# dpkn31/Yade-OpenFOAM-coupling

Hardware: AMD Instinct MI355X
Metric: coupled_steps_per_sec (pimpleFoamYade 4-way, 10M particles / 4M cells per GPU) (higher is better)
Workload: dtype f64

## Files before the change

yade-openfoam-coupling_amd/csrc/common.hpp:

```cpp
#pragma once
#include <hip/hip_runtime.h>

#include <algorithm>
#include <cmath>
#include <cstdarg>
#include <cstdint>
#include <cstdio>
#include <cstring>
#include <string>
#include <vector>

#include "../../include/foamyade_hip.h"

namespace fy {

struct Options {
    std::string tree_cache_dir;
    int rebin_interval;
    int strip_blocks;
    bool halo_overlap;
    int ipc_slot_mb;
    long long ipc_timeout_ms;
    bool wire_trace;
    bool explicit_tree;
    bool no_locate_lists;
    int locate_stack;
    bool locate_wide;
    bool no_deep_vcycle;
    long long mg_replicate_below;
    int amg_passes;
    bool localcomm_stream;
    bool no_fused_corrector;
    bool faces_from_arrays;
    bool no_pairs;
    bool no_tail_cache;
    int ipc_slot_kb;
};
Options options();

std::string& last_error();
int fail(int code, const char* fmt, ...);
bool pairs_disabled();
bool tail_cache_disabled();
bool locate_wide_forced();

#define FY_HIP(expr)                                                                                      \
    do {                                                                                                  \
        hipError_t _e = (expr);                                                                           \
        if (_e != hipSuccess)                                                                             \
            return ::fy::fail(FY_ERR_HIP, "%s failed: %s (%s:%d)", #expr, hipGetErrorString(_e), __FILE__, __LINE__); \
    } while (0)

#define FY_TRY(expr)                 \
    do {                             \
        int _rc = (expr);            \
        if (_rc != FY_OK) return _rc; \
// ... 203 lines not shown
```

yade-openfoam-coupling_amd/csrc/coupling.cpp:

```cpp
#include "coupling.hpp"
#include "ldu.hpp"

#include <algorithm>
#include <cmath>
#include <chrono>
#include <cstdlib>
#include <functional>
#include <thread>

#include <sys/stat.h>
#include <unistd.h>

#include <atomic>

namespace fy {

static std::atomic<int> g_kernel_flags{-1};
static bool kernel_flag(int bit) {
    if (g_kernel_flags.load(std::memory_order_relaxed) < 0) (void)options();
    return (g_kernel_flags.load(std::memory_order_relaxed) >> bit) & 1;
}
bool pairs_disabled() { return kernel_flag(0); }
bool tail_cache_disabled() { return kernel_flag(1); }
bool locate_wide_forced() { return kernel_flag(2); }

Options options() {
    auto on = [](const char* nm) { const char* e = getenv(nm); return e != nullptr && *e != 0 && strcmp(e, "0") != 0; };
    auto num = [](const char* nm, long long unset) { const char* e = getenv(nm); return e ? atoll(e) : unset; };
    Options q{};
    if (const char* d = getenv("FOAMYADE_TREE_CACHE_DIR")) q.tree_cache_dir = d;
    q.rebin_interval = std::max(1, (int)num("FOAMYADE_REBIN_INTERVAL", 32));
    q.strip_blocks = (int)num("FOAMYADE_STRIP_BLOCKS", -1);
    q.halo_overlap = getenv("FOAMYADE_HALO_OVERLAP") == nullptr || on("FOAMYADE_HALO_OVERLAP");
    q.ipc_slot_mb = (int)num("FOAMYADE_IPC_SLOT_MB", 0);
    q.ipc_timeout_ms = num("FOAMYADE_IPC_TIMEOUT_MS", 0);
    q.wire_trace = getenv("FOAMYADE_WIRE_TRACE") != nullptr;
    q.explicit_tree = on("FOAMYADE_EXPLICIT_TREE");
    q.no_locate_lists = on("FOAMYADE_NO_LOCATE_LISTS");
    q.locate_stack = (int)num("FOAMYADE_LOCATE_STACK", -1);
    q.locate_wide = num("FOAMYADE_LOCATE_WIDE", 0) != 0;
    q.no_deep_vcycle = on("FOAMYADE_NO_DEEP_VCYCLE");
    q.mg_replicate_below = std::max(0LL, num("FOAMYADE_MG_REPLICATE_BELOW", 0));
    q.amg_passes = (int)std::min(3LL, std::max(1LL, num("FOAMYADE_AMG_PASSES", 3)));
    const char* ls = getenv("FOAMYADE_LOCALCOMM_STREAM");
    q.localcomm_stream = ls != nullptr && ls[0] == '1';
    q.no_fused_corrector = on("FOAMYADE_NO_FUSED_CORRECTOR");
    q.faces_from_arrays = on("FOAMYADE_FACES_FROM_ARRAYS");
    q.no_pairs = on("FOAMYADE_NO_PAIRS");
    q.no_tail_cache = on("FOAMYADE_NO_TAIL_CACHE");
    q.ipc_slot_kb = (int)num("FOAMYADE_IPC_SLOT_KB", 0);
    g_kernel_flags.store((q.no_pairs ? 1 : 0) | (q.no_tail_cache ? 2 : 0) | (q.locate_wide ? 4 : 0), std::memory_order_relaxed);
    return q;
}

std::string& last_error() {
    static thread_local std::string e;
    return e;
}

int fail(int code, const char* fmt, ...) {
    char buf[1024];
    va_list ap;
    va_start(ap, fmt);
    vsnprintf(buf, sizeof(buf), fmt, ap);
    va_end(ap);
    last_error() = buf;
    return code;
}

static const int TAG_SZ_BUFF = 1003, TAG_GRID_BBOX = 1001, TAG_YADE_DATA = 1002, TAG_FORCE = 1005, TAG_SEARCH_RES = 1004,
// ... 1368 lines not shown
```

yade-openfoam-coupling_amd/csrc/fv_kernels.hip:

```cpp
#include "fv_kernels.hpp"

#include "common.hpp"
#include "device_util.hpp"
#include "fv_closures.hpp"

#ifndef FY_FVK_GRADED
#define FY_FVK_GRADED 0
#endif

namespace fy {
#if FY_FVK_GRADED
namespace gr {
#endif
namespace {

constexpr double kSmall = 1e-15;

__device__ __forceinline__ void ijk_of(const FvGeo& g, int t, int& i, int& j, int& k) {
    i = t % g.nx;
    const int q = t / g.nx;
    j = q % g.ny;
    k = q / g.ny;
}
__device__ __forceinline__ int cidx(const FvGeo& g, int i, int j, int k) { return i + g.nx * (j + g.ny * (k + g.gz)); }
// ... 377 lines not shown
    int i, j, k; ijk_of(g, t, i, j, k);
#define FY_CALL(D, fi, fj, fk) { const size_t f = (size_t)fid(g, D, fi, fj, fk); \
        flux_correct_face<D>(g, f, fi, fj, fk, p, phiHbyA.a[D], rAUf.a[D], alphaf.a[D], psn.a[D], phiForces.a[D], pflux.a[D], phi.a[D]); }
    FY_CELL_FACES(g, i, j, k, FY_CALL);
#undef FY_CALL
}

__global__ __launch_bounds__(256) void k_courant(FvGeo g, CFace3 phi, double* __restrict__ partials) {
    double v[2] = {0.0, 0.0};
    FY_RED_LOOP_G(g, t) {
        int i, j, k; ijk_of(g, t, i, j, k);
        double s = 0.0;
#pragma unroll
        for (int d = 0; d < 3; ++d)
#pragma unroll
            for (int sd = 0; sd < 2; ++sd) s += fabs(phi.a[d][cface(g, d, sd, i, j, k)]);
        v[0] = fmax(v[0], s * geo_rV(g, i, j, k));
        v[1] += s;
    }
    const int mx[2] = {1, 0};
    block_reduce_store<2>(v, mx, partials, fy_lb, fy_stride);
}

__global__ __launch_bounds__(256) void k_pre_coupling(FvGeo g, const double* __restrict__ U, const double* __restrict__ p,
                                                      const double* __restrict__ alpha, CFace3 psn, double* __restrict__ vGrad,
                                                      double* __restrict__ gradP, double* __restrict__ divT, double* __restrict__ Gout,
                                                      int write_vgrad, int write_pfields, CFace3 phi, double* __restrict__ ddtU, double* __restrict__ Uold_out,
                                                      double* __restrict__ cellrec, double rec_two_nu, double rec_rhoF, Face3 dcorr) {
    const int t = fv_block(g, blockIdx.x, gridDim.x) * 256 + (int)threadIdx.x;
    if (t >= g.Nc) return;
    int i, j, k; ijk_of(g, t, i, j, k);
    const int c = t + g.c0;
    const bool pf = g.pimple && write_pfields;
    const int ijk[3] = {i, j, k};
    bool bnd[3][2];
#pragma unroll
    for (int d = 0; d < 3; ++d)
#pragma unroll
        for (int s = 0; s < 2; ++s) bnd[d][s] = onb(g, d, s, i, j, k);
    const double uc[3] = {U[3 * (size_t)c], U[3 * (size_t)c + 1], U[3 * (size_t)c + 2]};
    const double pc = pf ? p[c] : 0.0, ac = pf ? alpha[c] : 0.0;
    double un6[3][2][3], pn6[3][2], an6[3][2];
#pragma unroll
    for (int d = 1; d < 3; ++d)
#pragma unroll
        for (int s = 0; s < 2; ++s) {
// ... 8 lines not shown
#pragma unroll
        for (int s = 0; s < 2; ++s) phf[d][s] = want_phi ? phi.a[d][cface(g, d, s, i, j, k)] : 0.0;
    const int lane = threadIdx.x & 63;
    {
        const int xm = (lane == 0 && i > 0) ? c - 1 : c, xp = (lane == 63 && i + 1 < g.nx) ? c + 1 : c;
        double em[3] = {0, 0, 0}, ep[3] = {0, 0, 0}, epm = 0, epp = 0, eam = 0, eap = 0;
        if (lane == 0 || lane == 63) {
            for (int q = 0; q < 3; ++q) { em[q] = U[3 * (size_t)xm + q]; ep[q] = U[3 * (size_t)xp + q]; }
            if (pf) { epm = p[xm]; epp = p[xp]; eam = alpha[xm]; eap = alpha[xp]; }
        }
#pragma unroll
        for (int q = 0; q < 3; ++q) { un6[0][0][q] = wave_prev(uc[q]); un6[0][1][q] = wave_next(uc[q]); }
        pn6[0][0] = wave_prev(pc); pn6[0][1] = wave_next(pc); an6[0][0] = wave_prev(ac); an6[0][1] = wave_next(ac);
        if (lane == 0 && i > 0) { for (int q = 0; q < 3; ++q) un6[0][0][q] = em[q]; pn6[0][0] = epm; an6[0][0] = eam; }
        if (lane == 63 && i + 1 < g.nx) { for (int q = 0; q < 3; ++q) un6[0][1][q] = ep[q]; pn6[0][1] = epp; an6[0][1] = eap; }
    }
    if (Uold_out) { Uold_out[3 * (size_t)c] = uc[0]; Uold_out[3 * (size_t)c + 1] = uc[1]; Uold_out[3 * (size_t)c + 2] = uc[2]; }
    double lap[3] = {0, 0, 0}, T[9], conv[3] = {0, 0, 0}, gp3[3] = {0, 0, 0};
#pragma unroll
    for (int d = 0; d < 3; ++d) {
        double fv[2][3], fp[2] = {0, 0};
#pragma unroll
        for (int s = 0; s < 2; ++s) {
            if (bnd[d][s]) {
                const int patch = 2 * d + s;
                if (g.u_bc[patch] == 0) { fv[s][0] = g.u_val[patch][0]; fv[s][1] = g.u_val[patch][1]; fv[s][2] = g.u_val[patch][2]; }
                else { fv[s][0] = uc[0]; fv[s][1] = uc[1]; fv[s][2] = uc[2]; }
                if (g.u_bc[patch] == 2) fv[s][d] = 0.0;
                if (pf) {
                    fp[s] = pbv(g, p, psn, c, d, s, cface(g, d, s, i, j, k));
                    for (int q = 0; q < 3; ++q) lap[q] += 1.0 * geo_Af(g, d, i, j, k) * (fv[s][q] - uc[q]) * geo_rhalf(g, d, ijk[d]);
                }
            } else {
                const double* un = un6[d][s];
                const int qc = ijk[d];
                for (int q = 0; q < 3; ++q) fv[s][q] = geo_lerp_side(g, d, s, qc, uc[q], un[q]);
                if (pf) {
                    fp[s] = geo_lerp_side(g, d, s, qc, pc, pn6[d][s]);
                    const double af = geo_lerp_side(g, d, s, qc, ac, an6[d][s]);
                    for (int q = 0; q < 3; ++q) lap[q] += af * geo_Af(g, d, i, j, k) * (un[q] - uc[q]) * geo_rdelta(g, d, qc + s);
                }
            }
        }
        if (dcorr.a[0]) {
#pragma unroll
            for (int s = 0; s < 2; ++s)
                if (owns_face(g, d, s, i, j, k)) {
                    const int fi = i + (d == 0 ? s : 0), fj = j + (d == 1 ? s : 0), fk = k + (d == 2 ? s : 0);
                    const int f = cface(g, d, s, i, j, k);
                    const double uf = fv[s][d] * geo_Af(g, d, fi, fj, fk);
                    const double po = phf[d][s];
                    const double phiCorr = po - uf;
                    const bool fixes = bnd[d][s] && g.u_bc[2 * d + s] == 0;
                    const double coef = fixes ? 0.0 : 1.0 - fmin(fabs(phiCorr) / (fabs(po) + kSmall), 1.0);
                    dcorr.a[d][f] = coef * (1.0 / g.dt) * phiCorr;
                }
        }
        const double rhd = geo_rh(g, d, ijk[d]);
        for (int q = 0; q < 3; ++q) T[3 * d + q] = (fv[1][q] - fv[0][q]) * rhd;
        if (pf) gp3[d] = (fp[1] - fp[0]) * rhd;
        if (ddtU) {
#pragma unroll
            for (int s = 0; s < 2; ++s) {
                const double flux = (s ? 1.0 : -1.0) * phf[d][s];
                for (int q = 0; q < 3; ++q) conv[q] += flux * fv[s][q];
            }
        }
    }
    if (ddtU)
        for (int q = 0; q < 3; ++q) ddtU[3 * (size_t)c + q] = conv[q] * geo_rV(g, i, j, k);
    if (write_vgrad)
        for (int q = 0; q < 9; ++q) vGrad[9 * (size_t)c + q] = T[q];
    if (pf)
        for (int q = 0; q < 3; ++q) gradP[3 * (size_t)c + q] = gp3[q];
    if (pf) {
        double dT[3];
        for (int q = 0; q < 3; ++q) { dT[q] = 2 * g.nu * (lap[q] * geo_rV(g, i, j, k)); divT[3 * (size_t)c + q] = dT[q]; }
        if (cellrec) {
            double2* r = reinterpret_cast<double2*>(cellrec + 8 * (size_t)c);
            r[0] = make_double2(uc[0], uc[1]);
            r[1] = make_double2(uc[2], ac);
            r[2] = make_double2(((rec_two_nu * dT[0]) * rec_rhoF) - gp3[0], ((rec_two_nu * dT[1]) * rec_rhoF) - gp3[1]);
            r[3] = make_double2(((rec_two_nu * dT[2]) * rec_rhoF) - gp3[2], geo_V(g, i, j, k));
        }
    }
    if (Gout) {
        const double tr = T[0] + T[4] + T[8];
        const double an = g.nut ? alpha[c] * (g.nu + g.nut[c]) : alpha[c] * g.nu;
        const size_t rs = g_row_stride(g);
        for (int a = 0; a < 3; ++a)
            for (int b = 0; b < 3; ++b) Gout[(size_t)a * rs + 3 * (size_t)c + b] = an * (T[3 * b + a] - (a == b ? (2.0 / 3.0) * tr : 0.0));
    }
}

__global__ __launch_bounds__(256) void k_div_G(FvGeo g, const double* __restrict__ G, double* __restrict__ divG) {
    const int t = fv_block(g, blockIdx.x, gridDim.x) * 256 + (int)threadIdx.x;
    if (t >= g.Nc) return;
    int i, j, k; ijk_of(g, t, i, j, k);
    const int c = t + g.c0;
    const int ijk[3] = {i, j, k};
    const double g0[3] = {G[3 * (size_t)c], G[3 * (size_t)c + 1], G[3 * (size_t)c + 2]};
    double gx[2][3];
    x_neighbours3(G, c, i, g.nx, g0, gx[0], gx[1]);
    bool bnd[3][2];
    double own[3][3], nbv[3][2][3];
#pragma unroll
    for (int q = 0; q < 3; ++q) { own[0][q] = g0[q]; nbv[0][0][q] = gx[0][q]; nbv[0][1][q] = gx[1][q]; }
#pragma unroll
    for (int d = 0; d < 3; ++d)
#pragma unroll
        for (int s = 0; s < 2; ++s) bnd[d][s] = onb(g, d, s, i, j, k);
#pragma unroll
    for (int d = 1; d < 3; ++d) {
        const double* Gd = G + (size_t)d * g_row_stride(g);
#pragma unroll
        for (int q = 0; q < 3; ++q) own[d][q] = Gd[3 * (size_t)c + q];
#pragma unroll
        for (int s = 0; s < 2; ++s) {
            const int nb = bnd[d][s] ? c : c + (s ? stride_of(g, d) : -stride_of(g, d));
#pragma unroll
            for (int q = 0; q < 3; ++q) nbv[d][s][q] = Gd[3 * (size_t)nb + q];
        }
    }
    double acc[3] = {0, 0, 0};
#pragma unroll
    for (int d = 0; d < 3; ++d) {
        double fv[2][3];
#pragma unroll
        for (int s = 0; s < 2; ++s)
            for (int q = 0; q < 3; ++q) fv[s][q] = bnd[d][s] ? own[d][q] : geo_lerp_side(g, d, s, ijk[d], own[d][q], nbv[d][s][q]);
        for (int q = 0; q < 3; ++q) acc[q] += (fv[1][q] - fv[0][q]) * geo_rh(g, d, ijk[d]);
    }
    for (int q = 0; q < 3; ++q) divG[3 * (size_t)c + q] = acc[q];
}

__global__ __launch_bounds__(256) void k_smagorinsky_nut(FvGeo g, const double* __restrict__ vGrad, double ck, double ce, double delta, double* __restrict__ nut) {
    const int t = blockIdx.x * 256 + threadIdx.x;
    if (t >= g.Nc) return;
    const int c = t + g.c0;
    delta = geo_delta(g, delta, c);
    double T[9];
#pragma unroll
    for (int q = 0; q < 9; ++q) T[q] = vGrad[9 * (size_t)c + q];
    nut[c] = smagorinsky_nut(T, ck, ce, delta);
}

__device__ __forceinline__ double wall_epsilon(const FvGeo& g, const TurbEqn& e, double kc, int c, int i, int j, int k) {
#if FY_FVK_GRADED
    double sum = 0.0;
    int W = 0;
#pragma unroll
    for (int d = 0; d < 3; ++d)
#pragma unroll
        for (int s = 0; s < 2; ++s)
            if (e.wall[2 * d + s] && onb(g, d, s, i, j, k)) { sum += wall_epsilon_term(e.cmu75, kc, e.kappa, geo_ywall(g, d, c)); ++W; }
// ... 949 lines not shown
}

int launch_pre_coupling(hipStream_t s, FvGeo g, const double* U, const double* p, const double* alpha, CFace3 psn, double* vGrad,
                        double* gradP, double* divT, double* Gout, int write_vgrad, int write_pfields, CFace3 phi, double* ddtU, double* Uold_out,
                        double* cellrec, double rec_nu, double rec_rhoF, Face3 dcorr) {
    hipLaunchKernelGGL(k_pre_coupling, dim3(fv_grid(g)), dim3(256), 0, s, g, U, p, alpha, psn, vGrad, gradP, divT, Gout, write_vgrad, write_pfields,
                       phi, ddtU, Uold_out, cellrec, 2.0 * rec_nu, rec_rhoF, dcorr);
    FY_LAUNCH_CHECK();
    return FY_OK;
}

int launch_interp_alpha(hipStream_t s, FvGeo g, const double* alpha, Face3 af) {
    hipLaunchKernelGGL(k_interp_alpha_cells, dim3(fv_grid(g)), dim3(256), 0, s, g, alpha, af);
    FY_LAUNCH_CHECK();
    return FY_OK;
}

int launch_div_G(hipStream_t s, FvGeo g, const double* G, double* divG) {
    hipLaunchKernelGGL(k_div_G, dim3(fv_grid(g)), dim3(256), 0, s, g, G, divG);
    FY_LAUNCH_CHECK();
    return FY_OK;
}

int launch_assemble_turb(hipStream_t s, FvGeo g, TurbEqn e, const double* k, const double* eps, const double* alpha, CFace3 alphaf, CFace3 phi,
                         const double* vGrad, const double* U, Mom7 M, double* b3, double* x3) {
    hipLaunchKernelGGL(k_assemble_turb, dim3(fv_grid(g)), dim3(256), 0, s, g, e, k, eps, alpha, alphaf, phi, vGrad, U, M, b3, x3);
    FY_LAUNCH_CHECK();
    return FY_OK;
}

int launch_turb_finish(hipStream_t s, FvGeo g, TurbEqn e, const double* x3, double* X, int nut_mode, double cmu, const double* eps, double* nut) {
    hipLaunchKernelGGL(k_turb_finish, dim3(fv_grid(g)), dim3(256), 0, s, g, e, x3, X, nut_mode, cmu, eps, nut);
    FY_LAUNCH_CHECK();
    return FY_OK;
}

int launch_assemble_scalar(hipStream_t s, FvGeo g, ScalarEqn e, const double* T, const double* alpha, CFace3 phi, const double* Sp, const double* Su, Mom7 M,
                           double* b3, double* x3) {
    hipLaunchKernelGGL(k_assemble_scalar, dim3(fv_grid(g)), dim3(256), 0, s, g, e, T, alpha, phi, Sp, Su, M, b3, x3);
    FY_LAUNCH_CHECK();
    return FY_OK;
}

int launch_scalar_finish(hipStream_t s, FvGeo g, const double* x3, double* X) {
    hipLaunchKernelGGL(k_scalar_finish, dim3(fv_grid(g)), dim3(256), 0, s, g, x3, X);
    FY_LAUNCH_CHECK();
// ... 173 lines not shown
```

yade-openfoam-coupling_amd/csrc/fv_kernels_api.inc:

```

int launch_flux_of(hipStream_t s, FvGeo g, const double* F, Face3 out);
int launch_courant(hipStream_t s, FvGeo g, CFace3 phi, double* partials);
int launch_pre_coupling(hipStream_t s, FvGeo g, const double* U, const double* p, const double* alpha, CFace3 psn,
                        double* vGrad, double* gradP, double* divT, double* Gout, int write_vgrad, int write_pfields,
                        CFace3 phi = CFace3{}, double* ddtU = nullptr, double* Uold_out = nullptr,
                        double* cellrec = nullptr ,
                        double rec_nu = 0.0, double rec_rhoF = 0.0,
                        Face3 dcorr = Face3{} );
int launch_interp_alpha(hipStream_t s, FvGeo g, const double* alpha, Face3 alphaf);
int launch_div_G(hipStream_t s, FvGeo g, const double* G, double* divG);
int launch_assemble_turb(hipStream_t s, FvGeo g, TurbEqn e, const double* k, const double* eps, const double* alpha, CFace3 alphaf, CFace3 phi,
                         const double* vGrad, const double* U, Mom7 M, double* b3, double* x3);
int launch_turb_finish(hipStream_t s, FvGeo g, TurbEqn e, const double* x3, double* X, int nut_mode, double cmu, const double* eps, double* nut);
int launch_assemble_scalar(hipStream_t s, FvGeo g, ScalarEqn e, const double* T, const double* alpha, CFace3 phi, const double* Sp, const double* Su, Mom7 M,
                           double* b3, double* x3);
int launch_scalar_finish(hipStream_t s, FvGeo g, const double* x3, double* X);
int launch_smagorinsky_nut(hipStream_t s, FvGeo g, const double* vGrad, double ck, double ce, double delta, double* nut);
int launch_assemble_momentum(hipStream_t s, FvGeo g, const double* U, const double* Uold, const double* alpha, const double* alphaOld,
                             CFace3 alphaf, CFace3 phi, const double* uSource, const double* uSourceDrag, const double* divG,
                             const double* vGrad , Mom7 M, double* src, double* rAU);
int launch_grad_magsqr(hipStream_t s, FvGeo g, const double* U, double* gradL);
int launch_interp_rAU(hipStream_t s, FvGeo g, const double* rAU, Face3 rAUf);
int launch_adjust_phi_sums(hipStream_t s, FvGeo g, CFace3 phiHbyA, CFace3 phiForces, double* partials);
int launch_adjust_phi_apply(hipStream_t s, FvGeo g, const double* sums, Face3 phiHbyA, CFace3 phiForces, CFace3 rAUf, const double* U, Face3 psn, int* err);
int launch_rAUf_phi_forces(hipStream_t s, FvGeo g, const double* rAU, const double* uSource, Face3 rf, Face3 out);
int launch_bmom(hipStream_t s, FvGeo g, const double* src, const double* p, CFace3 psn, CFace3 phiForces, CFace3 rAUf, double* bmom);
int launch_bmom_faces(hipStream_t s, FvGeo g, const double* rAU, const double* uSource, const double* src, const double* p, CFace3 psn, Face3 rAUf_out,
                      Face3 phiForces, double* bmom);
int launch_mom_pass(hipStream_t s, FvGeo g, Mom7 M, const double* b, const double* x, double* xn, const double* xsum ,
                    double n_glob, double* partials, const double* hsrc = nullptr, const double* rAU = nullptr, double* HbyA = nullptr);
int launch_HbyA(hipStream_t s, FvGeo g, Mom7 M, const double* src, const double* U, const double* rAU, double* HbyA);
int launch_phiHbyA(hipStream_t s, FvGeo g, const double* HbyA, const double* U, const double* Uold, CFace3 phiOld, CFace3 rAUf,
                   CFace3 alphaf, CFace3 phiForces, Face3 phiHbyA, Face3 psn, Face3 ddtc = Face3{} ,
// ... 22 lines not shown
```

yade-openfoam-coupling_amd/csrc/fv_solver.cpp:

```cpp
#include "fv_solver.hpp"

namespace fy {

int Solver::create(const fy_case_desc* c, const fy_transport* tr, int dev, Comm* cm) {
    if (c && (c->convection_scheme < FY_CONVECTION_LINEAR || c->convection_scheme > FY_CONVECTION_QUICK)) return fail(FY_ERR_INVALID, "fy_solver_create: unknown convection_scheme");
    if (c && c->convection_scheme == FY_CONVECTION_LIMITED_LINEAR && !(c->convection_limiter_k >= 0 && c->convection_limiter_k <= 1)) return fail(FY_ERR_INVALID, "fy_solver_create: limitedLinear's coefficient must lie in [0, 1]");
    const bool gradedc = c && (c->hx || c->hy || c->hz);
    if (!c || c->nx <= 0 || c->ny <= 0 || c->nz <= 0 || (!gradedc && !(c->dx > 0)) || !(c->dt > 0)) return fail(FY_ERR_INVALID, "fy_solver_create: bad case");
    if (gradedc) {
        if (!(c->hx && c->hy && c->hz)) return fail(FY_ERR_INVALID, "fy_solver_create: a graded block needs hx, hy AND hz");
        if (cm && cm->size > 1) return fail(FY_ERR_UNSUPPORTED, "fy_solver_create: z-slabs need the uniform block (a graded block runs on one domain)");
        const double* hh[3] = {c->hx, c->hy, c->hz};
        const int nn[3] = {c->nx, c->ny, c->nz};
        for (int a = 0; a < 3; ++a) for (int q = 0; q < nn[a]; ++q) if (!(hh[a][q] > 0)) return fail(FY_ERR_INVALID, "fy_solver_create: graded block with a non-positive cell size");
    }
    if (c->thermal.on && cm && cm->size > 1)
        return fail(FY_ERR_UNSUPPORTED, "fy_solver_create_slab: heat transfer (fy_case_desc.thermal.on) is not available on z-slabs (%d ranks; foamYadeHip_mpi -parallel): "
                                        "run the case on one domain", cm->size);
    int ndev = 0;
    if (hipGetDeviceCount(&ndev) != hipSuccess || ndev == 0) return fail(FY_ERR_NO_DEVICE, "no HIP device visible: libfoamyade_hip has no CPU path");
    if (dev < 0 || dev >= ndev) return fail(FY_ERR_INVALID, "device ordinal out of range");
    cs = *c; device = dev; pimple = c->solver == FY_SOLVER_PIMPLE;
    cs.hx = cs.hy = cs.hz = nullptr;
    comm = cm ? cm : &self_comm;
// ... 128 lines not shown
            if (c->u_bc[q] == FY_BC_U_SLIP) continue;
            if (c->u_bc[q] != FY_BC_U_FIXED_VALUE) { adjustable = true; continue; }
            const double un = c->u_value[q][q / 2] * ((q & 1) ? 1.0 : -1.0) * area[q / 2];
            net += un; mag += std::fabs(un);
        }
        if (!adjustable && std::fabs(net) > 1e-8 * (mag + 1e-300))
            return fail(FY_ERR_UNSUPPORTED, "no patch fixes the pressure and the fixed-value velocity patches do not balance (net flux %g of %g): OpenFOAM's adjustPhi "
                                            "ends such a run with 'Continuity error cannot be removed by adjusting the outflow'", net, mag);
        adjust_phi = adjustable || mag > 0.0;
    }

    const size_t n = nstore;
    DevBuf<double>* v3[] = {&U, &Uold, &uSource, &uParticle, &gradP, &divT, &ddtU, &src, &HbyA, &bmom, &divG, &xscr};
    for (auto* b : v3) { FY_TRY(b->alloc_exact(3 * n)); FY_TRY(zero(*b)); }
    DevBuf<double>* v1[] = {&p, &alpha, &uSourceDrag, &mdiag, &rAU, &prhs, &pr, &pw, &pp, &ps, &pzj};
    for (auto* b : v1) { FY_TRY(b->alloc_exact(n)); FY_TRY(zero(*b)); }
    for (auto& b : man) { FY_TRY(b.alloc_exact(n)); FY_TRY(zero(b)); }
    for (int q = 0; q < 6; ++q) if (c->u_bc[q] == FY_BC_U_SLIP && !mbd.p) { FY_TRY(mbd.alloc_exact(3 * n)); FY_TRY(zero(mbd)); }
    FY_TRY(vGrad.alloc_exact(9 * n)); FY_TRY(zero(vGrad));
    if (c->convection_scheme >= FY_CONVECTION_LIMITED_LINEAR) { FY_TRY(gradL.alloc_exact(3 * n)); FY_TRY(zero(gradL)); }
    if (c->turbulence_model != FY_TURBULENCE_LAMINAR) { FY_TRY(nut.alloc_exact(n)); FY_TRY(launch_fill_f64(stream, nut.p, n, c->nut_initial)); g.nut = nut.p; }
    if (c->turbulence_model == FY_TURBULENCE_KEQN || c->turbulence_model == FY_TURBULENCE_KEPSILON) { FY_TRY(kturb.alloc_exact(n)); FY_TRY(launch_fill_f64(stream, kturb.p, n, c->k_initial)); g.kturb = kturb.p; }
    if (c->turbulence_model == FY_TURBULENCE_KEPSILON) { FY_TRY(epsturb.alloc_exact(n)); FY_TRY(launch_fill_f64(stream, epsturb.p, n, c->eps_initial)); g.epsturb = epsturb.p; }
    FY_TRY(Gt.alloc_exact(9 * n)); FY_TRY(zero(Gt));
    for (int d = 0; d < 3; ++d) {
        DevBuf<double>* fs[] = {&phi[d], &phiOld[d], &psn[d], &alphaf[d], &phiHbyA[d], &phiForces[d], &rAUf[d], &pflux[d], &ddtc[d], &dcorr[d]};
        for (auto* b : fs) { FY_TRY(b->alloc_exact(fv_fsize(g, d))); FY_TRY(zero(*b)); }
        FY_TRY(launch_fill_f64(stream, alphaf[d].p, alphaf[d].n, 1.0));
    }
    FY_TRY(launch_fill_f64(stream, alpha.p, n, 1.0));
    FY_TRY(launch_fill_f64(stream, rAU.p, n, 1.0));
    FY_TRY(partials.alloc_exact(8 * (size_t)red_blocks(Nc))); FY_TRY(red_out.alloc_exact(8)); FY_TRY(sc.alloc_exact(8)); FY_TRY(xbar3.alloc_exact(3));
    FY_TRY(zero(partials)); FY_TRY(zero(sc)); FY_TRY(zero(red_out));
    if (adjust_phi) { FY_TRY(adj_sums.alloc_exact(4)); FY_TRY(adj_err.alloc_exact(1)); FY_HIP(hipMemsetAsync(adj_err.p, 0, sizeof(int), stream)); }
    rb.init(kDeferBase + kDeferMax);
    FY_TRY(ops_courant.alloc_exact(2));
    FY_TRY(ops_diag.alloc_exact(4));
    { const int h4[4] = {0, 0, 1, 0}; FY_HIP(hipMemcpyAsync(ops_diag.p, h4, sizeof(h4), hipMemcpyHostToDevice, stream)); }
    { const int h[2] = {1, 0}; FY_HIP(hipMemcpyAsync(ops_courant.p, h, sizeof(h), hipMemcpyHostToDevice, stream)); FY_HIP(hipStreamSynchronize(stream)); }

    {
        int ax = g.nx, ay = g.ny, az_loc = g.nz, az_glob = c->nz;
        bool dist = S > 1;
        size_t lvl = 0;
        const int64_t replicate_below = opt.mg_replicate_below > 0 ? (int64_t)opt.mg_replicate_below : (int64_t)kMgReplicateBelow;
        mg_rep = (size_t)-1;
        for (;;) {
// ... 475 lines not shown
        const int rc = cpl->c.set_particle_action(cs.dt);
        cpl->c.mid_hook = nullptr; cpl->c.mid_hook_user = nullptr;
        FY_TRY(rc);
    }
    if (timing) { tim[0].stop(stream); }
    if (th.on) FY_TRY(heat_coefficients());
    if (th.buoyant) FY_TRY(buoyancy());
    const double* usrc = momentum_source();
    comm->tag = "momentum";

    if (pimple && face_arrays) FY_TRY(FVK(launch_interp_alpha, stream, g, alpha.p, F3(alphaf)));
    const int nOuter = pimple ? std::max(cs.n_outer_correctors, 1) : 1;
    for (int outer = 0; outer < nOuter; ++outer) {
        const bool final_outer = outer == nOuter - 1;
        g.u_relax = (final_outer && cs.u_relax_final > 0) ? cs.u_relax_final : cs.u_relax;
        p_relax_now = (final_outer && cs.p_relax_final > 0) ? cs.p_relax_final : cs.p_relax;
        if (pimple && p_relax_now > 0 && p_relax_now < 1) {
            if (!pPrev.p) FY_TRY(pPrev.alloc_exact(nstore));
            FY_TRY(launch_copy_f64(stream, pPrev.p, p.p, nstore));
        }
        clk_mom.begin(stream);
        if (pimple) {
            if (outer > 0) FY_TRY(halo_U());
            FY_TRY(FVK(launch_pre_coupling, stream, g, U.p, p.p, alpha.p, C3(psn), vGrad.p, gradP.p, divT.p, Gt.p, g.upwind == 2 ? 1 : 0, 0));
            FY_TRY(overlapped(XW_MOMENTUM, true, [&](hipStream_t on) { return halo(Gt.p + 2 * 3 * nstore, 3, plane, g.nz, g.gz, 1, on); },
                              [&](const FvGeo& gw) { return FVK(launch_div_G, stream, gw, Gt.p, divG.p); }));
        }
        if (g.upwind == 2) FY_TRY(halo_cells(vGrad, 9, 1));
        if (g.upwind >= 3) {
            FY_TRY(halo_U());
            FY_TRY(FVK(launch_grad_magsqr, stream, g, U.p, gradL.p));
            FY_TRY(halo_cells(gradL, 3, 1));
        }
        FY_TRY(FVK(launch_assemble_momentum, stream, g, U.p, Uold.p, alpha.p,  alpha.p, face_arrays ? C3(alphaf) : CFace3{}, phi_now(), usrc, uSourceDrag.p,
                                        divG.p, g.upwind >= 3 ? gradL.p : vGrad.p, M7(), src.p, rAU.p));
        rAU_new = true; hbya_ready = false;
        const bool bmom_fused = pimple && cs.momentum_predictor && fused_corrector;
        if (pimple) {
            if (cpl->c.slab.tail_pending) { FY_HIP(hipStreamWaitEvent(stream, cpl->c.slab.ev_tail, 0)); cpl->c.slab.tail_pending = false; }
            if (bmom_fused) {
                FY_TRY(overlapped(XW_MOMENTUM, true, [&](hipStream_t on) { return halo_cells(rAU, 1, 1, on); }, [&](const FvGeo& gw) {
                    return FVK(launch_bmom_faces, stream, gw, rAU.p, usrc, src.p, p.p, C3(psn), face_arrays ? F3(rAUf) : Face3{}, F3(phiForces), bmom.p);
                }));
            } else {
                FY_TRY(halo_cells(rAU, 1, 1));
                FY_TRY(FVK(launch_rAUf_phi_forces, stream, g, rAU.p, usrc, F3(rAUf), F3(phiForces)));
            }
        }
        if (cs.momentum_predictor) {
// ... 31 lines not shown
        clk_mom.collect(); clk_pres.collect();
        st.ms_momentum = clk_mom.total_ms; st.ms_pressure = clk_pres.total_ms;
        st.ms_particle = tim[0].ms() - cpl->c.marks.ms(6, 7);
        st.ms_total = tim[3].ms();
        st.ms_other = st.ms_total - st.ms_particle - st.ms_momentum - st.ms_pressure;
        for (auto& k : kc) k.collect();
        avg.clock.collect(); mon.clock.collect();
        if (th.on) { th.clk_coeff.collect(); th.clk_flux.collect(); th.clk_asm.collect(); th.clk_buoy.collect(); }
        if (ss.on) ss.clock.collect();
    }
    if (xwait_timing) {
        for (auto& k : clk_xwait) k.collect();
    }
    return FY_OK;
}

int Solver::field(const char* name, double** ptr, size_t* count) {
    const std::string s = name ? name : "";
    const size_t n = (size_t)Nc;
    struct E { const char* nm; double* p; size_t c; int comp; };
    const E tab[] = {{"U", U.p, 3 * n, 3}, {"p", p.p, n, 1}, {"phi_x", phi[0].p, phi[0].n, 0}, {"phi_y", phi[1].p, phi[1].n, 0}, {"phi_z", phi[2].p, phi[2].n, 0},
                     {"rAU", rAU.p, n, 1}, {"HbyA", HbyA.p, 3 * n, 3}, {"p_rhs", prhs.p, n, 1}, {"mom_diag", mdiag.p, n, 1}, {"mom_src", src.p, 3 * n, 3},
                     {"alpha", alpha.p, n, 1}, {"uSource", uSource.p, 3 * n, 3}, {"uSourceDrag", uSourceDrag.p, n, 1}, {"uParticle", uParticle.p, 3 * n, 3},
                     {"gradP", gradP.p, 3 * n, 3}, {"divT", divT.p, 3 * n, 3}, {"vGrad", vGrad.p, 9 * n, 9}, {"ddtU", ddtU.p, 3 * n, 3}, {"nut", nut.p, n, 1}, {"k", kturb.p, n, 1}, {"epsilon", epsturb.p, n, 1}};
    if (s == "T" || s == "heatSp" || s == "heatSu") {
        if (!th.on) return fail(FY_ERR_INVALID, "solver field '%s' does not exist in this case (fy_case_desc.thermal is off)", s.c_str());
        *ptr = (s == "T" ? th.T.p : s == "heatSp" ? th.Sp.p : th.Su.p) + g.c0;
        *count = n;
        return FY_OK;
    }
    if (s == "buoyancy") {
        if (!th.buoyant) return fail(FY_ERR_INVALID, "solver field 'buoyancy' does not exist in this case (fy_case_desc.thermal.beta or g is zero)");
        *ptr = th.buoy.p + 3 * (size_t)g.c0;
        *count = 3 * n;
        return FY_OK;
    }
    for (const E& e : tab) if (s == e.nm) {
        if (!e.p) return fail(FY_ERR_INVALID, "solver field '%s' does not exist in this case (no turbulence model)", s.c_str());
        const bool transport = cs.turbulence_model == FY_TURBULENCE_KEQN || cs.turbulence_model == FY_TURBULENCE_KEPSILON;
        if (th.on && (s == "HbyA" || s == "mom_diag"))
            return fail(FY_ERR_UNSUPPORTED, "solver field '%s' is overwritten by the temperature solve in this case (the T equation reuses the momentum matrix's storage)", s.c_str());
        if (transport && (s == "HbyA" || s == "mom_diag" || s == "mom_src"))
            return fail(FY_ERR_UNSUPPORTED, "solver field '%s' is overwritten by the turbulence transport solve in this case (kEqn / kEpsilon reuse the momentum matrix's storage)", s.c_str());
        *ptr = e.p + (size_t)e.comp * g.c0;
        *count = e.c;
        return FY_OK;
    }
    MgLev& L = *mg[0];
    const struct { const char* nm; double* p; } pm[] = {{"p_diag", L.diag.p}, {"p_ux", L.ux.p}, {"p_uy", L.uy.p}, {"p_uz", L.uz.p}};
    for (auto& e : pm) if (s == e.nm) { *ptr = e.p + L.A.c0; *count = n; return FY_OK; }
    if (s.size() > 2 && s.compare(0, 2, "mg") == 0 && s[2] >= '1' && s[2] <= '9') {
        size_t q = 2, lvl = 0;
        while (q < s.size() && s[q] >= '0' && s[q] <= '9' && lvl < 1000) lvl = 10 * lvl + (size_t)(s[q++] - '0');
        const std::string arr = s.substr(q);
        if (lvl < mg.size() && (arr == "_diag" || arr == "_ux" || arr == "_uy" || arr == "_uz")) {
            MgLev& M = *mg[lvl];
            double* base = arr == "_diag" ? M.diag.p : arr == "_ux" ? M.ux.p : arr == "_uy" ? M.uy.p : M.uz.p;
// ... 29 lines not shown
```

yade-openfoam-coupling_amd/csrc/fv_solver.hpp:

```cpp
#pragma once
#include <algorithm>
#include <cmath>
#include <memory>
#include <string>
#include <functional>
#include <vector>

#include "comm.hpp"
#include "coupling.hpp"
#include "field_average.hpp"
#include "fv_kernels.hpp"
#include "heat_exchange.hpp"
#include "solid_stats.hpp"

#define FVK(fn, ...) (g.graded ? ::fy::gr::fn(__VA_ARGS__) : ::fy::fn(__VA_ARGS__))

namespace fy {

constexpr int kMgCoarsest = kMgDirectMax, kMgCoarsestEdge = 8;
constexpr int kMgDeepGhost = 5;
constexpr int kMgReplicateBelow = 1 << 20;

struct MgLev {
    PMat A{};
// ... 173 lines not shown
    int smooth(size_t l, MgLev& L, double w, bool with_dot = false);
    PMat slice_of(const MgLev& L, const MgLev& Cc) const;
    static constexpr double kMgWa = 1.7318685872766142, kMgWb = 0.5695012757370842;
    MgWeights mgw{2, {kMgWa, kMgWb, 0, 0}};
    int vcycle(size_t l);
    PMat planes_of(const MgLev& L, int ext, int* kofs = nullptr) const;
    int vcycle_deep(size_t l, int E);
    int exchange_operator_ghosts(MgLev& L);
    bool want_vcycle_dot = false, vcycle_dot_done = false;
    static constexpr int kMgCoarseSweeps = 120;
    int coarse_sweeps = kMgCoarseSweeps;
    bool fuse_prolong = true;
    int ref_cell_at(size_t lvl, const PMat& A, int k0) const;
    int build_coarse_operators();
    DevBuf<double> mg_inv, mg_ref;
    double p_sum = 0.0;
    bool p_sum_valid = false;
    int solve_pressure(bool final_iter, bool init_done = false);
    int precondition(const double* r_host, double* z_host);
    int prepare_p_init(bool with_halo = true);
    bool fused_corrector = true;
    bool hbya_ready = false;
    bool face_arrays = true;
    bool faces_from_cells = true;

    int corrector(bool final_inner);
    bool fuse_diag = true;
    int carry_slot = -1;
    bool carry_valid = false;
    double carry_h[2] = {0, 0};

    std::vector<int> cont_slots;
    int courant_slot = -1;
    void note_cont_err(const double* h) {
        const double tv = total_volume;
        st.cont_err_sum_local = cs.dt * h[0] / tv; st.cont_err_global = cs.dt * h[1] / tv;
        cumulative_cont_err += st.cont_err_global; st.cont_err_cumulative = cumulative_cont_err;
    }
    void note_courant(const double* h) { st.courant_max = 0.5 * h[0] * cs.dt; st.courant_mean = 0.5 * (h[1] / total_volume) * cs.dt; }
    int turbulence_correct();
    int st_k_iters = 0;

    int step();
    FieldAverage avg;
    const double* avg_source(const std::string& name, int* comp) const;
    int set_field_average(const fy_average_desc* d);
// ... 25 lines not shown
```

Measured before the change: 196.2.

## Fuse stress tensor build and divergence into one LDS-tiled kernel

```diff
diff --git a/yade-openfoam-coupling_amd/csrc/common.hpp b/yade-openfoam-coupling_amd/csrc/common.hpp
--- a/yade-openfoam-coupling_amd/csrc/common.hpp
+++ b/yade-openfoam-coupling_amd/csrc/common.hpp
@@ -32,6 +32,7 @@
     bool localcomm_stream;
     bool no_fused_corrector;
     bool faces_from_arrays;
+    bool no_tiled_stress;
     bool no_pairs;
     bool no_tail_cache;
     int ipc_slot_kb;
diff --git a/yade-openfoam-coupling_amd/csrc/coupling.cpp b/yade-openfoam-coupling_amd/csrc/coupling.cpp
--- a/yade-openfoam-coupling_amd/csrc/coupling.cpp
+++ b/yade-openfoam-coupling_amd/csrc/coupling.cpp
@@ -46,6 +46,7 @@
     q.localcomm_stream = ls != nullptr && ls[0] == '1';
     q.no_fused_corrector = on("FOAMYADE_NO_FUSED_CORRECTOR");
     q.faces_from_arrays = on("FOAMYADE_FACES_FROM_ARRAYS");
+    q.no_tiled_stress = on("FOAMYADE_NO_TILED_STRESS");
     q.no_pairs = on("FOAMYADE_NO_PAIRS");
     q.no_tail_cache = on("FOAMYADE_NO_TAIL_CACHE");
     q.ipc_slot_kb = (int)num("FOAMYADE_IPC_SLOT_KB", 0);
diff --git a/yade-openfoam-coupling_amd/csrc/fv_kernels.hip b/yade-openfoam-coupling_amd/csrc/fv_kernels.hip
--- a/yade-openfoam-coupling_amd/csrc/fv_kernels.hip
+++ b/yade-openfoam-coupling_amd/csrc/fv_kernels.hip
@@ -423,6 +423,35 @@
     block_reduce_store<2>(v, mx, partials, fy_lb, fy_stride);
 }
 
+__device__ __forceinline__ void u_face_value(const FvGeo& g, int d, int s, bool on_boundary, int qc, const double (&uc)[3], const double* un, double (&fv)[3]) {
+    if (on_boundary) {
+        const int patch = 2 * d + s;
+        if (g.u_bc[patch] == 0) { fv[0] = g.u_val[patch][0]; fv[1] = g.u_val[patch][1]; fv[2] = g.u_val[patch][2]; }
+        else { fv[0] = uc[0]; fv[1] = uc[1]; fv[2] = uc[2]; }
+        if (g.u_bc[patch] == 2) fv[d] = 0.0;
+    } else {
+        for (int q = 0; q < 3; ++q) fv[q] = geo_lerp_side(g, d, s, qc, uc[q], un[q]);
+    }
+}
+__device__ __forceinline__ void grad_row(const FvGeo& g, int d, int qc, const double (&fv)[2][3], double (&T)[9]) {
+    const double rhd = geo_rh(g, d, qc);
+    for (int q = 0; q < 3; ++q) T[3 * d + q] = (fv[1][q] - fv[0][q]) * rhd;
+}
+__device__ __forceinline__ double stress_trace(const double (&T)[9]) { return T[0] + T[4] + T[8]; }
+__device__ __forceinline__ double stress_coeff(const FvGeo& g, const double* __restrict__ alpha, int c) { return g.nut ? alpha[c] * (g.nu + g.nut[c]) : alpha[c] * g.nu; }
+__device__ __forceinline__ double stress_entry(double an, const double (&T)[9], double tr, int a, int b) { return an * (T[3 * b + a] - (a == b ? (2.0 / 3.0) * tr : 0.0)); }
+__device__ __forceinline__ void div_of_rows(const FvGeo& g, const bool (&bnd)[3][2], const int (&ijk)[3], const double (&own)[3][3], const double (&nbv)[3][2][3], double (&acc)[3]) {
+    acc[0] = acc[1] = acc[2] = 0.0;
+#pragma unroll
+    for (int d = 0; d < 3; ++d) {
+        double fv[2][3];
+#pragma unroll
+        for (int s = 0; s < 2; ++s)
+            for (int q = 0; q < 3; ++q) fv[s][q] = bnd[d][s] ? own[d][q] : geo_lerp_side(g, d, s, ijk[d], own[d][q], nbv[d][s][q]);
+        for (int q = 0; q < 3; ++q) acc[q] += (fv[1][q] - fv[0][q]) * geo_rh(g, d, ijk[d]);
+    }
+}
+
 __global__ __launch_bounds__(256) void k_pre_coupling(FvGeo g, const double* __restrict__ U, const double* __restrict__ p,
                                                       const double* __restrict__ alpha, CFace3 psn, double* __restrict__ vGrad,
                                                       double* __restrict__ gradP, double* __restrict__ divT, double* __restrict__ Gout,
@@ -477,11 +506,8 @@
         double fv[2][3], fp[2] = {0, 0};
 #pragma unroll
         for (int s = 0; s < 2; ++s) {
+            u_face_value(g, d, s, bnd[d][s], ijk[d], uc, un6[d][s], fv[s]);
             if (bnd[d][s]) {
-                const int patch = 2 * d + s;
-                if (g.u_bc[patch] == 0) { fv[s][0] = g.u_val[patch][0]; fv[s][1] = g.u_val[patch][1]; fv[s][2] = g.u_val[patch][2]; }
-                else { fv[s][0] = uc[0]; fv[s][1] = uc[1]; fv[s][2] = uc[2]; }
-                if (g.u_bc[patch] == 2) fv[s][d] = 0.0;
                 if (pf) {
                     fp[s] = pbv(g, p, psn, c, d, s, cface(g, d, s, i, j, k));
                     for (int q = 0; q < 3; ++q) lap[q] += 1.0 * geo_Af(g, d, i, j, k) * (fv[s][q] - uc[q]) * geo_rhalf(g, d, ijk[d]);
@@ -489,7 +515,6 @@
             } else {
                 const double* un = un6[d][s];
                 const int qc = ijk[d];
-                for (int q = 0; q < 3; ++q) fv[s][q] = geo_lerp_side(g, d, s, qc, uc[q], un[q]);
                 if (pf) {
                     fp[s] = geo_lerp_side(g, d, s, qc, pc, pn6[d][s]);
                     const double af = geo_lerp_side(g, d, s, qc, ac, an6[d][s]);
@@ -511,9 +536,8 @@
                     dcorr.a[d][f] = coef * (1.0 / g.dt) * phiCorr;
                 }
         }
-        const double rhd = geo_rh(g, d, ijk[d]);
-        for (int q = 0; q < 3; ++q) T[3 * d + q] = (fv[1][q] - fv[0][q]) * rhd;
-        if (pf) gp3[d] = (fp[1] - fp[0]) * rhd;
+        grad_row(g, d, ijk[d], fv, T);
+        if (pf) gp3[d] = (fp[1] - fp[0]) * geo_rh(g, d, ijk[d]);
         if (ddtU) {
 #pragma unroll
             for (int s = 0; s < 2; ++s) {
@@ -540,11 +564,11 @@
         }
     }
     if (Gout) {
-        const double tr = T[0] + T[4] + T[8];
-        const double an = g.nut ? alpha[c] * (g.nu + g.nut[c]) : alpha[c] * g.nu;
+        const double tr = stress_trace(T);
+        const double an = stress_coeff(g, alpha, c);
         const size_t rs = g_row_stride(g);
         for (int a = 0; a < 3; ++a)
-            for (int b = 0; b < 3; ++b) Gout[(size_t)a * rs + 3 * (size_t)c + b] = an * (T[3 * b + a] - (a == b ? (2.0 / 3.0) * tr : 0.0));
+            for (int b = 0; b < 3; ++b) Gout[(size_t)a * rs + 3 * (size_t)c + b] = stress_entry(an, T, tr, a, b);
     }
 }
 
@@ -577,15 +601,123 @@
             for (int q = 0; q < 3; ++q) nbv[d][s][q] = Gd[3 * (size_t)nb + q];
         }
     }
-    double acc[3] = {0, 0, 0};
+    double acc[3];
+    div_of_rows(g, bnd, ijk, own, nbv, acc);
+    for (int q = 0; q < 3; ++q) divG[3 * (size_t)c + q] = acc[q];
+}
+
+#ifndef FY_STRESS_TILE_X
+#define FY_STRESS_TILE_X 16
+#endif
+#ifndef FY_STRESS_TILE_Y
+#define FY_STRESS_TILE_Y 8
+#endif
+#ifndef FY_STRESS_TILE_Z
+#define FY_STRESS_TILE_Z 4
+#endif
+constexpr int kSTX = FY_STRESS_TILE_X, kSTY = FY_STRESS_TILE_Y, kSTZ = FY_STRESS_TILE_Z;
+constexpr int kStressThreads = kSTX * kSTY * kSTZ;
+constexpr int kSlabX = 2 * kSTY * kSTZ, kSlabY = 2 * kSTX * kSTZ, kSlabZ = 2 * kSTX * kSTY;
+static_assert(kStressThreads % 64 == 0 && kStressThreads <= 1024, "a tile is a whole number of waves and one workgroup");
+static_assert(((kSTX + 2) * kSTY * kSTZ + kSTX * (kSTY + 2) * kSTZ + kSTX * kSTY * (kSTZ + 2)) * 3 * sizeof(double) <= 64 * 1024, "the tile's rows fit static LDS");
+
+template <unsigned ROWS>
+__device__ __forceinline__ void stress_rows_at(const FvGeo& g, const double* __restrict__ U, const double* __restrict__ alpha, int i, int j, int k, double (&G)[3][3]) {
+    const int c = cidx(g, i, j, k);
+    const int ijk[3] = {i, j, k};
+    const double uc[3] = {U[3 * (size_t)c], U[3 * (size_t)c + 1], U[3 * (size_t)c + 2]};
+    bool bnd[3][2];
+    double un6[3][2][3];
+#pragma unroll
+    for (int d = 0; d < 3; ++d)
+#pragma unroll
+        for (int s = 0; s < 2; ++s) {
+            bnd[d][s] = onb(g, d, s, i, j, k);
+            const int nb = bnd[d][s] ? c : c + (s ? stride_of(g, d) : -stride_of(g, d));
+            un6[d][s][0] = U[3 * (size_t)nb]; un6[d][s][1] = U[3 * (size_t)nb + 1]; un6[d][s][2] = U[3 * (size_t)nb + 2];
+        }
+    double T[9];
 #pragma unroll
     for (int d = 0; d < 3; ++d) {
         double fv[2][3];
 #pragma unroll
-        for (int s = 0; s < 2; ++s)
-            for (int q = 0; q < 3; ++q) fv[s][q] = bnd[d][s] ? own[d][q] : geo_lerp_side(g, d, s, ijk[d], own[d][q], nbv[d][s][q]);
-        for (int q = 0; q < 3; ++q) acc[q] += (fv[1][q] - fv[0][q]) * geo_rh(g, d, ijk[d]);
-    }
+        for (int s = 0; s < 2; ++s) u_face_value(g, d, s, bnd[d][s], ijk[d], uc, un6[d][s], fv[s]);
+        grad_row(g, d, ijk[d], fv, T);
+    }
+    const double tr = stress_trace(T);
+    const double an = stress_coeff(g, alpha, c);
+#pragma unroll
+    for (int a = 0; a < 3; ++a)
+        if ((ROWS >> a) & 1)
+            for (int b = 0; b < 3; ++b) G[a][b] = stress_entry(an, T, tr, a, b);
+}
+
+__global__ __launch_bounds__(kStressThreads) void k_stress_div(FvGeo g, const double* __restrict__ U, const double* __restrict__ alpha, double* __restrict__ divG, int ntx, int nty) {
+    __shared__ double sx[3][(kSTX + 2) * kSTY * kSTZ], sy[3][kSTX * (kSTY + 2) * kSTZ], sz[3][kSTX * kSTY * (kSTZ + 2)];
+    const int tile = swz_block(blockIdx.x, gridDim.x);
+    const int tq = tile / ntx;
+    const int i0 = (tile - tq * ntx) * kSTX, j0 = (tq % nty) * kSTY, k0 = (tq / nty) * kSTZ;
+    const int tid = threadIdx.x;
+    const int lx = tid % kSTX, ly = (tid / kSTX) % kSTY, lz = tid / (kSTX * kSTY);
+    const int i = i0 + lx, j = j0 + ly, k = k0 + lz;
+    const bool in = i < g.nx && j < g.ny && k < g.nz;
+    const int ex = (lx + 1) + (kSTX + 2) * (ly + kSTY * lz), ey = lx + kSTX * ((ly + 1) + (kSTY + 2) * lz), ez = lx + kSTX * (ly + kSTY * (lz + 1));
+    double own[3][3];
+    if (in) {
+        stress_rows_at<7u>(g, U, alpha, i, j, k, own);
+#pragma unroll
+        for (int q = 0; q < 3; ++q) { sx[q][ex] = own[0][q]; sy[q][ey] = own[1][q]; sz[q][ez] = own[2][q]; }
+    }
+    for (int h = tid; h < kSlabX + kSlabY + kSlabZ; h += kStressThreads) {
+        double G[3][3];
+        if (h < kSlabX) {
+            const int s = h / (kSTY * kSTZ), r = h - s * (kSTY * kSTZ), hy = r % kSTY, hz = r / kSTY;
+            const int hi = s ? i0 + kSTX : i0 - 1, hj = j0 + hy, hk = k0 + hz;
+            if (hi >= 0 && hi < g.nx && hj < g.ny && hk < g.nz) {
+                stress_rows_at<1u>(g, U, alpha, hi, hj, hk, G);
+#pragma unroll
+                for (int q = 0; q < 3; ++q) sx[q][(s ? kSTX + 1 : 0) + (kSTX + 2) * (hy + kSTY * hz)] = G[0][q];
+            }
+        } else if (h < kSlabX + kSlabY) {
+            const int hh = h - kSlabX;
+            const int s = hh / (kSTX * kSTZ), r = hh - s * (kSTX * kSTZ), hx = r % kSTX, hz = r / kSTX;
+            const int hi = i0 + hx, hj = s ? j0 + kSTY : j0 - 1, hk = k0 + hz;
+            if (hj >= 0 && hj < g.ny && hi < g.nx && hk < g.nz) {
+                stress_rows_at<2u>(g, U, alpha, hi, hj, hk, G);
+#pragma unroll
+                for (int q = 0; q < 3; ++q) sy[q][hx + kSTX * ((s ? kSTY + 1 : 0) + (kSTY + 2) * hz)] = G[1][q];
+            }
+        } else {
+            const int hh = h - kSlabX - kSlabY;
+            const int s = hh / (kSTX * kSTY), r = hh - s * (kSTX * kSTY), hx = r % kSTX, hy = r / kSTX;
+            const int hi = i0 + hx, hj = j0 + hy, hk = s ? k0 + kSTZ : k0 - 1;
+            if (hk >= 0 && hk < g.nz && hi < g.nx && hj < g.ny) {
+                stress_rows_at<4u>(g, U, alpha, hi, hj, hk, G);
+#pragma unroll
+                for (int q = 0; q < 3; ++q) sz[q][hx + kSTX * (hy + kSTY * (s ? kSTZ + 1 : 0))] = G[2][q];
+            }
+        }
+    }
+    __syncthreads();
+    if (!in) return;
+    const int ijk[3] = {i, j, k};
+    bool bnd[3][2];
+    double nbv[3][2][3];
+#pragma unroll
+    for (int d = 0; d < 3; ++d)
+#pragma unroll
+        for (int s = 0; s < 2; ++s) bnd[d][s] = onb(g, d, s, i, j, k);
+#pragma unroll
+    for (int s = 0; s < 2; ++s) {
+        const int nx_ = bnd[0][s] ? ex : ex + (s ? 1 : -1);
+        const int ny_ = bnd[1][s] ? ey : ey + (s ? kSTX : -kSTX);
+        const int nz_ = bnd[2][s] ? ez : ez + (s ? kSTX * kSTY : -kSTX * kSTY);
+#pragma unroll
+        for (int q = 0; q < 3; ++q) { nbv[0][s][q] = sx[q][nx_]; nbv[1][s][q] = sy[q][ny_]; nbv[2][s][q] = sz[q][nz_]; }
+    }
+    double acc[3];
+    div_of_rows(g, bnd, ijk, own, nbv, acc);
+    const int c = cidx(g, i, j, k);
     for (int q = 0; q < 3; ++q) divG[3 * (size_t)c + q] = acc[q];
 }
 
@@ -1581,6 +1713,14 @@
     return FY_OK;
 }
 
+int launch_stress_div(hipStream_t s, FvGeo g, const double* U, const double* alpha, double* divG) {
+    if (g.gz != 0 || g.c0 != 0 || g.win_nblk > 0) return fail(FY_ERR_INVALID, "launch_stress_div: single domain only (a slab exchanges row z of G between the two sweeps)");
+    const int ntx = (int)div_up(g.nx, kSTX), nty = (int)div_up(g.ny, kSTY), ntz = (int)div_up(g.nz, kSTZ);
+    hipLaunchKernelGGL(k_stress_div, dim3((unsigned)(ntx * nty * ntz)), dim3(kStressThreads), 0, s, g, U, alpha, divG, ntx, nty);
+    FY_LAUNCH_CHECK();
+    return FY_OK;
+}
+
 int launch_assemble_turb(hipStream_t s, FvGeo g, TurbEqn e, const double* k, const double* eps, const double* alpha, CFace3 alphaf, CFace3 phi,
                          const double* vGrad, const double* U, Mom7 M, double* b3, double* x3) {
     hipLaunchKernelGGL(k_assemble_turb, dim3(fv_grid(g)), dim3(256), 0, s, g, e, k, eps, alpha, alphaf, phi, vGrad, U, M, b3, x3);
diff --git a/yade-openfoam-coupling_amd/csrc/fv_kernels_api.inc b/yade-openfoam-coupling_amd/csrc/fv_kernels_api.inc
--- a/yade-openfoam-coupling_amd/csrc/fv_kernels_api.inc
+++ b/yade-openfoam-coupling_amd/csrc/fv_kernels_api.inc
@@ -9,6 +9,7 @@
                         Face3 dcorr = Face3{} );
 int launch_interp_alpha(hipStream_t s, FvGeo g, const double* alpha, Face3 alphaf);
 int launch_div_G(hipStream_t s, FvGeo g, const double* G, double* divG);
+int launch_stress_div(hipStream_t s, FvGeo g, const double* U, const double* alpha, double* divG);
 int launch_assemble_turb(hipStream_t s, FvGeo g, TurbEqn e, const double* k, const double* eps, const double* alpha, CFace3 alphaf, CFace3 phi,
                          const double* vGrad, const double* U, Mom7 M, double* b3, double* x3);
 int launch_turb_finish(hipStream_t s, FvGeo g, TurbEqn e, const double* x3, double* X, int nut_mode, double cmu, const double* eps, double* nut);
diff --git a/yade-openfoam-coupling_amd/csrc/fv_solver.cpp b/yade-openfoam-coupling_amd/csrc/fv_solver.cpp
--- a/yade-openfoam-coupling_amd/csrc/fv_solver.cpp
+++ b/yade-openfoam-coupling_amd/csrc/fv_solver.cpp
@@ -174,7 +174,8 @@
     if (c->turbulence_model != FY_TURBULENCE_LAMINAR) { FY_TRY(nut.alloc_exact(n)); FY_TRY(launch_fill_f64(stream, nut.p, n, c->nut_initial)); g.nut = nut.p; }
     if (c->turbulence_model == FY_TURBULENCE_KEQN || c->turbulence_model == FY_TURBULENCE_KEPSILON) { FY_TRY(kturb.alloc_exact(n)); FY_TRY(launch_fill_f64(stream, kturb.p, n, c->k_initial)); g.kturb = kturb.p; }
     if (c->turbulence_model == FY_TURBULENCE_KEPSILON) { FY_TRY(epsturb.alloc_exact(n)); FY_TRY(launch_fill_f64(stream, epsturb.p, n, c->eps_initial)); g.epsturb = epsturb.p; }
-    FY_TRY(Gt.alloc_exact(9 * n)); FY_TRY(zero(Gt));
+    tiled_stress = pimple && S == 1 && g.upwind != 2 && !opt.no_tiled_stress;
+    if (!tiled_stress) { FY_TRY(Gt.alloc_exact(9 * n)); FY_TRY(zero(Gt)); }
     for (int d = 0; d < 3; ++d) {
         DevBuf<double>* fs[] = {&phi[d], &phiOld[d], &psn[d], &alphaf[d], &phiHbyA[d], &phiForces[d], &rAUf[d], &pflux[d], &ddtc[d], &dcorr[d]};
         for (auto* b : fs) { FY_TRY(b->alloc_exact(fv_fsize(g, d))); FY_TRY(zero(*b)); }
@@ -696,9 +697,13 @@
         clk_mom.begin(stream);
         if (pimple) {
             if (outer > 0) FY_TRY(halo_U());
-            FY_TRY(FVK(launch_pre_coupling, stream, g, U.p, p.p, alpha.p, C3(psn), vGrad.p, gradP.p, divT.p, Gt.p, g.upwind == 2 ? 1 : 0, 0));
-            FY_TRY(overlapped(XW_MOMENTUM, true, [&](hipStream_t on) { return halo(Gt.p + 2 * 3 * nstore, 3, plane, g.nz, g.gz, 1, on); },
-                              [&](const FvGeo& gw) { return FVK(launch_div_G, stream, gw, Gt.p, divG.p); }));
+            if (tiled_stress) {
+                FY_TRY(FVK(launch_stress_div, stream, g, U.p, alpha.p, divG.p));
+            } else {
+                FY_TRY(FVK(launch_pre_coupling, stream, g, U.p, p.p, alpha.p, C3(psn), vGrad.p, gradP.p, divT.p, Gt.p, g.upwind == 2 ? 1 : 0, 0));
+                FY_TRY(overlapped(XW_MOMENTUM, true, [&](hipStream_t on) { return halo(Gt.p + 2 * 3 * nstore, 3, plane, g.nz, g.gz, 1, on); },
+                                  [&](const FvGeo& gw) { return FVK(launch_div_G, stream, gw, Gt.p, divG.p); }));
+            }
         }
         if (g.upwind == 2) FY_TRY(halo_cells(vGrad, 9, 1));
         if (g.upwind >= 3) {
@@ -776,7 +781,7 @@
     const E tab[] = {{"U", U.p, 3 * n, 3}, {"p", p.p, n, 1}, {"phi_x", phi[0].p, phi[0].n, 0}, {"phi_y", phi[1].p, phi[1].n, 0}, {"phi_z", phi[2].p, phi[2].n, 0},
                      {"rAU", rAU.p, n, 1}, {"HbyA", HbyA.p, 3 * n, 3}, {"p_rhs", prhs.p, n, 1}, {"mom_diag", mdiag.p, n, 1}, {"mom_src", src.p, 3 * n, 3},
                      {"alpha", alpha.p, n, 1}, {"uSource", uSource.p, 3 * n, 3}, {"uSourceDrag", uSourceDrag.p, n, 1}, {"uParticle", uParticle.p, 3 * n, 3},
-                     {"gradP", gradP.p, 3 * n, 3}, {"divT", divT.p, 3 * n, 3}, {"vGrad", vGrad.p, 9 * n, 9}, {"ddtU", ddtU.p, 3 * n, 3}, {"nut", nut.p, n, 1}, {"k", kturb.p, n, 1}, {"epsilon", epsturb.p, n, 1}};
+                     {"gradP", gradP.p, 3 * n, 3}, {"divT", divT.p, 3 * n, 3}, {"vGrad", vGrad.p, 9 * n, 9}, {"divG", divG.p, 3 * n, 3}, {"ddtU", ddtU.p, 3 * n, 3}, {"nut", nut.p, n, 1}, {"k", kturb.p, n, 1}, {"epsilon", epsturb.p, n, 1}};
     if (s == "T" || s == "heatSp" || s == "heatSu") {
         if (!th.on) return fail(FY_ERR_INVALID, "solver field '%s' does not exist in this case (fy_case_desc.thermal is off)", s.c_str());
         *ptr = (s == "T" ? th.T.p : s == "heatSp" ? th.Sp.p : th.Su.p) + g.c0;
@@ -787,6 +792,12 @@
         if (!th.buoyant) return fail(FY_ERR_INVALID, "solver field 'buoyancy' does not exist in this case (fy_case_desc.thermal.beta or g is zero)");
         *ptr = th.buoy.p + 3 * (size_t)g.c0;
         *count = 3 * n;
+        return FY_OK;
+    }
+    if (s == "stress_G") {
+        if (!Gt.p) return fail(FY_ERR_INVALID, "solver field 'stress_G' does not exist in this case (the tiled sweep keeps the tensor in LDS; FOAMYADE_NO_TILED_STRESS=1 stores it)");
+        *ptr = Gt.p;
+        *count = 9 * nstore;
         return FY_OK;
     }
     for (const E& e : tab) if (s == e.nm) {
diff --git a/yade-openfoam-coupling_amd/csrc/fv_solver.hpp b/yade-openfoam-coupling_amd/csrc/fv_solver.hpp
--- a/yade-openfoam-coupling_amd/csrc/fv_solver.hpp
+++ b/yade-openfoam-coupling_amd/csrc/fv_solver.hpp
@@ -219,6 +219,7 @@
     bool fused_corrector = true;
     bool hbya_ready = false;
     bool face_arrays = true;
+    bool tiled_stress = false;
     bool faces_from_cells = true;
 
     int corrector(bool final_inner);
```

Measured after the change: 199.9, median of 6. 1.9% higher.
